# shreyaspadhy/CMCD

Hardware: AMD Instinct MI355X
Metric: bridge-steps*particles/sec (higher is better)
Workload: dtype f32; 1 GPU; many_gmm_n2000_k256_dds; model=many_gmm, boundmode=MCD_CAIS_sn, particles_per_gpu=2000, nbridges=256, nn_arch=dds, dim=2, global_particles=2000, parallelism=particles sharded x1, stats all-gather

## Files before the change

### cmcd_amd/csrc/cmcd_kernels.hip

```cpp
#include <hip/hip_runtime.h>
#include <math.h>
#include <stdint.h>
#include <stdio.h>
#include <stdlib.h>
#include <string.h>

#include "cmcd_common.h"
#include "cmcd_device.h"
#include "cmcd_hip.h"
#include "cmcd_host.h"

namespace cmcd {

struct SchedArgs {
  const float* params;
  float* ws;
  cmcd_layout lay;
  WsLayout w;
  int32_t K, ngrid, eps_schedule;
  int64_t gridref_x, target_x;
  uint32_t stamp = 0;
};

__device__ __forceinline__ void prep_sched_body(const SchedArgs& a) {
  __shared__ float gy[40], gx[40], gm[40];
  const int G = a.ngrid;
  if (threadIdx.x <= G) gm[threadIdx.x] = a.params[a.lay.mgridref_y + threadIdx.x];
  __syncthreads();
  if (threadIdx.x == 0) {
    float v[33];
#pragma unroll
    for (int i = 0; i < 33; ++i) v[i] = gm[i < G + 1 ? i : G];
    float run = 0.f;
#pragma unroll
    for (int i = 0; i < 33; ++i) {
      if (i <= G) {
        run += v[i];
        gy[i + 1] = run;
      }
    }
    gy[0] = 0.f;
    gm[39] = run;
  }
  __syncthreads();
  if (threadIdx.x < G + 2) {
    const float tot = gm[39];
    if (threadIdx.x >= 1) gy[threadIdx.x] = gy[threadIdx.x] / tot;
    gx[threadIdx.x] = (float)threadIdx.x / (float)(G + 1);
  }
  __syncthreads();
  const float eps0 = a.params[a.lay.eps];
  for (int i = threadIdx.x; i < a.K; i += blockDim.x) {
    const float x = (float)(i + 1) / (float)(a.K + 1);
    int j = (int)(x * (float)(G + 1)) + 1;
    j = j < 1 ? 1 : (j > G + 1 ? G + 1 : j);
    while (j > 1 && gx[j - 1] > x) --j;
    while (j < G + 1 && gx[j] <= x) ++j;
    const float dx = gx[j] - gx[j - 1], df = gy[j] - gy[j - 1];
    a.ws[a.w.beta + i] = gy[j - 1] + ((x - gx[j - 1]) / dx) * df;
    float e;
    if (a.eps_schedule == CMCD_EPS_COS_SQ) {
      const float phase = (float)i / (float)a.K;
      const float cs = cosf((phase + 0.008f) / 1.008f * 0.5f * 3.14159265358979323846f);
      e = eps0 * (cs * cs);
    } else if (a.eps_schedule == CMCD_EPS_LINEAR) {
      e = (0.0001f - eps0) / (float)(a.K - 1) * (float)i + eps0;
    } else {
      e = eps0;
    }
    const float s = sqrtf(2.0f * e);
    a.ws[a.w.eps + i] = e;
    a.ws[a.w.sig + i] = s;
    a.ws[a.w.logsig + i] = logf(s);
    float* sc = a.ws + a.w.sched + 8 * (int64_t)i;
    sc[0] = a.ws[a.w.beta + i];
    sc[1] = e;
    sc[2] = s;
    sc[3] = logf(s) + kHalfLog2Pi;
    sc[4] = 1.0f / (2.0f * s * s);
    sc[5] = e * sc[0];
    sc[6] = e * (1.0f - sc[0]);
    sc[7] = i == 0 ? __uint_as_float(a.stamp) : 0.f;
  }
}

__global__ void prep_sched_kernel(SchedArgs a) { prep_sched_body(a); }

struct DdsPrepArgs {
  const float* params;
  float* ws;
  cmcd_layout lay;
  WsLayout w;
  int32_t D;
};

__device__ __forceinline__ void prep_dds_body(const DdsPrepArgs& a, int t) {
  __shared__ float e[128], h[64], tau[64], red[4][64];
  const int j = threadIdx.x & 63, q = threadIdx.x >> 6;
  const float* P = a.params;
  float wa[32], wb[16], wc[16];
#pragma unroll
  for (int k = 0; k < 32; ++k) wa[k] = P[a.lay.d_tw1 + (32 * q + k) * 64 + j];
#pragma unroll
  for (int k = 0; k < 16; ++k) wb[k] = P[a.lay.d_tw2 + (16 * q + k) * 64 + j];
#pragma unroll
  for (int k = 0; k < 16; ++k) wc[k] = P[a.lay.d_sw1 + (a.D + 16 * q + k) * 64 + j];
  const float ba = P[a.lay.d_tb1 + j], bb = P[a.lay.d_tb2 + j], bc = P[a.lay.d_sb1 + j];
  if (q == 0) {
    float cj;
    {
#pragma clang fp contract(off)
      const float sj = (float)j / 63.0f;
      const float lo_part = 0.1f * (1.0f - sj), hi_part = 100.0f * sj;
      cj = (j == 63) ? 100.0f : lo_part + hi_part;
    }
    const float arg = cj * (float)t + P[a.lay.d_phase + j];
    e[j] = sinf(arg);
    e[64 + j] = cosf(arg);
  }
  __syncthreads();
  float acc = 0.f;
#pragma unroll
  for (int k = 0; k < 32; ++k) acc = fmaf(e[32 * q + k], wa[k], acc);
  red[q][j] = acc;
  __syncthreads();
  if (q == 0) h[j] = gelu_exact(ba + ((red[0][j] + red[1][j]) + (red[2][j] + red[3][j])));
  __syncthreads();
  acc = 0.f;
#pragma unroll
  for (int k = 0; k < 16; ++k) acc = fmaf(h[16 * q + k], wb[k], acc);
  __syncthreads();
  red[q][j] = acc;
  __syncthreads();
  if (q == 0) tau[j] = bb + ((red[0][j] + red[1][j]) + (red[2][j] + red[3][j]));
  __syncthreads();
  acc = 0.f;
#pragma unroll
  for (int k = 0; k < 16; ++k) acc = fmaf(tau[16 * q + k], wc[k], acc);
  __syncthreads();
  red[q][j] = acc;
  __syncthreads();
  if (q == 0) a.ws[a.w.bias1 + (int64_t)t * 64 + j] = bc + ((red[0][j] + red[1][j]) + (red[2][j] + red[3][j]));
}

struct GefPrepArgs {
  const float* params;
  float* ws;
  cmcd_layout lay;
  WsLayout w;
  int32_t D, E, K;
};

__device__ __forceinline__ void prep_geffner_body(const GefPrepArgs& a, int row) {
  const int ie = row < a.K ? row : a.K - 1;
  const int in = a.D + a.E;
  const float* P = a.params;
  const float* emb = P + a.lay.g_emb + (int64_t)ie * a.E;
  for (int n = threadIdx.x; n < a.w.HP; n += blockDim.x) {
    float b = 0.f, u = 0.f;
    if (n < in) {
      b = P[a.lay.g_b1 + n];
      const float* wcol = P + a.lay.g_w1 + (int64_t)a.D * in + n;
      int j = 0;
      for (; j + 8 <= a.E; j += 8) {
        float wv[8];
#pragma unroll
        for (int q = 0; q < 8; ++q) wv[q] = wcol[(int64_t)(j + q) * in];
#pragma unroll
        for (int q = 0; q < 8; ++q) b = fmaf(emb[j + q], wv[q], b);
      }
      for (; j < a.E; ++j) b = fmaf(emb[j], wcol[(int64_t)j * in], b);
      u = n >= a.D ? emb[n - a.D] : 0.f;
    }
    a.ws[a.w.bias1 + (int64_t)row * a.w.HP + n] = b;
    a.ws[a.w.utab + (int64_t)row * a.w.HP + n] = u;
  }
}

struct PackArgs {
  const float* params;
  const float* tgt;
  float* ws;
  WsLayout w;
  int64_t o_w1, o_w2, o_b2, o_w3, o_b3, o_factor;
  int32_t D, IN;
  int32_t DO;
  int32_t target, n_mix;
  uint32_t stamp;
};

__device__ __forceinline__ void pack_weights_body(const PackArgs& a, int vblock, int nblocks) {
  const int HP = a.w.HP, T = a.w.T;
  const float* P = a.params;
  const int64_t tid = (int64_t)vblock * blockDim.x + threadIdx.x;
  const int64_t stride = (int64_t)nblocks * blockDim.x;
  const bool has_net = a.o_w2 >= 0;
  for (int64_t idx = tid; has_net && idx < (int64_t)HP * HP; idx += stride) {
    const int r = idx & 3, lane = (idx >> 2) & 63;
    const int tt = int(idx >> 8), t_out = tt % T, t_in = tt / T;
    const int kin = 16 * t_in + 4 * (lane >> 4) + r, nout = 16 * t_out + (lane & 15);
    a.ws[a.w.w2 + idx] = (kin < a.IN && nout < a.IN) ? P[a.o_w2 + (int64_t)kin * a.IN + nout] : 0.f;
    const int krow = 16 * t_in + (lane & 15), ncon = 16 * t_out + 4 * (lane >> 4) + r;
    a.ws[a.w.w2t + idx] = (krow < a.IN && ncon < a.IN) ? P[a.o_w2 + (int64_t)krow * a.IN + ncon] : 0.f;
  }
  for (int64_t idx = tid; has_net && idx < 2 * (int64_t)HP * HP; idx += stride) {
    const int lane = idx & 63, rest = int(idx >> 6), sq = rest % (HP / 2), wvq = rest / (HP / 2);
    int kin = sq + (HP / 2) * ((lane >> 3) & 1), nout = 16 * wvq + 4 * (lane >> 4) + (lane & 3);
    if (wvq == 8 && coop_tail4(T, a.IN)) {
      const int sl = (lane >> 3) & 7;
      kin = sq < coop_tail_len(sl) ? coop_tail_start(sl) + sq : a.IN;
      nout = 128 + (lane & 3);
    }
    a.ws[a.w.w2q + idx] = (kin < a.IN && nout < a.IN) ? P[a.o_w2 + (int64_t)kin * a.IN + nout] : 0.f;
  }
  for (int64_t idx = tid; has_net && idx < (int64_t)a.D * HP; idx += stride) {
    const int j = int(idx / HP), n = int(idx % HP);
    a.ws[a.w.w1z + idx] = n < a.IN ? P[a.o_w1 + (int64_t)j * a.IN + n] : 0.f;
  }
  for (int64_t idx = tid; has_net && idx < (int64_t)a.DO * HP; idx += stride) {
    const int j = int(idx / HP), n = int(idx % HP);
    a.ws[a.w.w3t + idx] = n < a.IN ? P[a.o_w3 + (int64_t)n * a.DO + j] : 0.f;
  }
  for (int64_t idx = tid; has_net && idx < HP; idx += stride) a.ws[a.w.b2 + idx] = idx < a.IN ? P[a.o_b2 + idx] : 0.f;
  for (int64_t idx = tid; idx < 16; idx += stride) {
    float v = 0.f;
    if (has_net && idx < a.DO) v = P[a.o_b3 + idx];
    if (idx == 15) v = a.o_factor >= 0 ? P[a.o_factor] : 1.0f;
    if (idx == 13) v = __uint_as_float(a.stamp);
    a.ws[a.w.b3 + idx] = v;
  }
  if (a.target == CMCD_TARGET_MANY_GMM) {
    for (int64_t idx = tid; idx < a.w.tgt_floats; idx += stride) {
      float v = 0.f;
      const float s = a.tgt[0];
      if (idx == 0) v = 1.0f / s;
      else if (idx == 1) v = -0.5f * 1.44269504088896340736f / (s * s);
      else if (idx == 2) v = __int_as_float(a.n_mix);
      else if (idx == 3) v = 1.44269504088896340736f * (-2.0f * (logf(s) + kHalfLog2Pi) - logf((float)a.n_mix));
      else if (idx >= 4 && idx < 4 + 2 * a.n_mix) v = a.tgt[1 + (idx - 4)];
      a.ws[a.w.tgt + idx] = v;
    }
  }
}

struct PrepArgs {
  SchedArgs sched;
  DdsPrepArgs dds;
  GefPrepArgs gef;
  PackArgs pack;
  int32_t K, arch, npack;
};

__global__ __launch_bounds__(256) void prep_fused_kernel(PrepArgs a) {
  const int b = blockIdx.x;
  if (b <= a.K) {
    if (a.arch < 0) return;
    if (a.arch == CMCD_ARCH_DDS) prep_dds_body(a.dds, b);
    else prep_geffner_body(a.gef, b);
  } else if (b == a.K + 1) {
    prep_sched_body(a.sched);
  } else {
    pack_weights_body(a.pack, b - a.K - 2, a.npack);
  }
}


template <int ARCH>
__device__ __forceinline__ float act(float pre) {
  return ARCH == CMCD_ARCH_DDS ? gelu_exact(pre) : softplus(pre);
}

#ifndef CMCD_TRAJ_ABL
#define CMCD_TRAJ_ABL 0
#endif
#ifndef CMCD_TRAJ_PF
#define CMCD_TRAJ_PF 1
#endif
template <int ARCH, int D, int T, bool PF = (CMCD_TRAJ_PF != 0)>
__device__ __forceinline__ void eval_net(const float (&z)[D], const float* __restrict__ brow,
                                         const float* __restrict__ urow, const float* lds_w2,
                                         const float* lds_w1z, const float* lds_b2, const float* lds_w3t,
                                         const float* lds_b3, int lane, float (&s)[D]) {
  constexpr int HP = 16 * T;
  const int g = lane >> 4;
  asm volatile("" ::: "memory");
  f32x4 h[T];
#pragma unroll
  for (int t = 0; t < T; ++t) {
    f32x4 pre = *reinterpret_cast<const f32x4*>(brow + 16 * t + 4 * g);
#pragma unroll
    for (int j = 0; j < D; ++j) {
      const f32x4 wv = *reinterpret_cast<const f32x4*>(lds_w1z + j * HP + 16 * t + 4 * g);
      pre += z[j] * wv;
    }
    if (ARCH == CMCD_ARCH_DDS) {
#pragma unroll
      for (int r = 0; r < 4; ++r) h[t][r] = (CMCD_TRAJ_ABL & 2) ? pre[r] : gelu_fast(pre[r]);
    } else {
      f32x4 u = *reinterpret_cast<const f32x4*>(urow + 16 * t + 4 * g);
      if (16 * t < D) {
#pragma unroll
        for (int r = 0; r < 4; ++r) {
          const int nidx = 16 * t + 4 * g + r;
#pragma unroll
          for (int j = 0; j < D; ++j)
            if (j >= 16 * t && j < 16 * t + 16) u[r] = (nidx == j) ? z[j] : u[r];
        }
      }
#pragma unroll
      for (int r = 0; r < 4; ++r) h[t][r] = u[r] + softplus(pre[r]);
    }
  }
  float dummy = z[0];
  f32x4 acc[T];
#pragma unroll
  for (int t = 0; t < T; ++t) acc[t] = *reinterpret_cast<const f32x4*>(lds_b2 + 16 * t + 4 * g);
  if (PF) {
    f32x4 a[2][T];
    asm volatile("" ::: "memory");
#pragma unroll
    for (int to = 0; to < T; ++to) a[0][to] = *reinterpret_cast<const f32x4*>(lds_w2 + (to * 64 + lane) * 4);
#pragma unroll
    for (int ti = 0; ti < T; ++ti) {
      asm volatile("" ::: "memory");
      if (ti + 1 < T) {
#pragma unroll
        for (int to = 0; to < T; ++to)
          a[(ti + 1) & 1][to] = *reinterpret_cast<const f32x4*>(lds_w2 + (((ti + 1) * T + to) * 64 + lane) * 4);
      }
      __builtin_amdgcn_sched_barrier(0);
#pragma unroll
      for (int r = 0; r < 4; ++r) {
#pragma unroll
        for (int to = 0; to < T; ++to)
          acc[to] = __builtin_amdgcn_mfma_f32_16x16x4f32(a[ti & 1][to][r], h[ti][r], acc[to], 0, 0, 0);
      }
      __builtin_amdgcn_sched_barrier(0);
    }
  } else {
#pragma unroll
  for (int ti = 0; ti < T; ++ti) {
    asm volatile("" ::: "memory");
    f32x4 a[T];
#pragma unroll
    for (int to = 0; to < T; ++to)
      a[to] = *reinterpret_cast<const f32x4*>(lds_w2 + ((ti * T + to) * 64 + lane) * 4);
#pragma unroll
    for (int r = 0; r < 4; ++r) {
#pragma unroll
      for (int to = 0; to < T; ++to) {
        if (CMCD_TRAJ_ABL & 1) acc[to][r] += a[to][r] * h[ti][r];
        else acc[to] = __builtin_amdgcn_mfma_f32_16x16x4f32(a[to][r], h[ti][r], acc[to], 0, 0, 0);
      }
      if (CMCD_TRAJ_ABL & 16) {
#pragma unroll
        for (int q = 0; q < 24; ++q) asm volatile("v_fma_f32 %0, %0, %1, %1" : "+v"(dummy) : "v"(z[0]));
      }
    }
  }
  }
  if (CMCD_TRAJ_ABL & 32) {
#pragma unroll
    for (int q = 0; q < 24 * 4 * T; ++q) asm volatile("v_fma_f32 %0, %0, %1, %1" : "+v"(dummy) : "v"(z[0]));
  }
  float part[D];
#pragma unroll
  for (int j = 0; j < D; ++j) part[j] = 0.f;
#pragma unroll
  for (int t = 0; t < T; ++t) {
    f32x4 h2;
#pragma unroll
    for (int r = 0; r < 4; ++r)
      h2[r] = (ARCH == CMCD_ARCH_DDS) ? ((CMCD_TRAJ_ABL & 2) ? acc[t][r] : gelu_fast(acc[t][r])) : h[t][r] + softplus(acc[t][r]);
#pragma unroll
    for (int j = 0; j < D; ++j) {
      const f32x4 wv = *reinterpret_cast<const f32x4*>(lds_w3t + j * HP + 16 * t + 4 * g);
      part[j] += h2[0] * wv[0] + h2[1] * wv[1] + h2[2] * wv[2] + h2[3] * wv[3];
    }
  }
  const float factor = lds_b3[15];
#pragma unroll
  for (int j = 0; j < D; ++j) {
    const float o = group_sum(part[j]) + lds_b3[j];
    s[j] = (ARCH == CMCD_ARCH_DDS) ? fminf(fmaxf(o, -1e4f), 1e4f) : o * factor;
  }
  if (CMCD_TRAJ_ABL & 48) s[0] += dummy * 1e-30f;
}

__device__ __forceinline__ float traj_rs32(float x, float y) {
  uint32_t r0, r1;
  swap32(__float_as_uint(x), __float_as_uint(y), r0, r1);
  return __uint_as_float(r0) + __uint_as_float(r1);
}
__device__ __forceinline__ float traj_rs16(float x, float y) {
  uint32_t r0, r1;
  swap16(__float_as_uint(x), __float_as_uint(y), r0, r1);
  return __uint_as_float(r0) + __uint_as_float(r1);
}
template <int ARCH, int D, int T>
__device__ __forceinline__ void eval_net_tail4(const float (&z)[D], const float* __restrict__ brow,
                                               const float* __restrict__ urow, const float* lds_w2,
                                               const float* lds_w1z, const float* lds_b2, const float* lds_w3t,
                                               const float* lds_b3, int lane, float (&s)[D]) {
  static_assert(ARCH == CMCD_ARCH_GEFFNER && T >= 2 && D <= 16, "the tail form is the geffner net's");
  constexpr int HP = 16 * T, TF = T - 1, NX = 16 * TF;
  const int g = lane >> 4, c = lane & 15;
  asm volatile("" ::: "memory");
  f32x4 h[TF];
#pragma unroll
  for (int t = 0; t < TF; ++t) {
    f32x4 pre = *reinterpret_cast<const f32x4*>(brow + 16 * t + 4 * g);
#pragma unroll
    for (int j = 0; j < D; ++j) {
      const f32x4 wv = *reinterpret_cast<const f32x4*>(lds_w1z + j * HP + 16 * t + 4 * g);
      pre += z[j] * wv;
    }
    f32x4 u = *reinterpret_cast<const f32x4*>(urow + 16 * t + 4 * g);
    if (16 * t < D) {
#pragma unroll
      for (int r = 0; r < 4; ++r) {
        const int nidx = 16 * t + 4 * g + r;
#pragma unroll
        for (int j = 0; j < D; ++j)
          if (j >= 16 * t && j < 16 * t + 16) u[r] = (nidx == j) ? z[j] : u[r];
      }
    }
#pragma unroll
    for (int r = 0; r < 4; ++r) h[t][r] = u[r] + softplus(pre[r]);
  }
  float hx;
  {
    float px = brow[NX + g];
#pragma unroll
    for (int j = 0; j < D; ++j) px = fmaf(z[j], lds_w1z[j * HP + NX + g], px);
    hx = urow[NX + g] + softplus(px);
  }
  f32x4 acc[TF], accx = {0.f, 0.f, 0.f, 0.f};
#pragma unroll
  for (int t = 0; t < TF; ++t) acc[t] = *reinterpret_cast<const f32x4*>(lds_b2 + 16 * t + 4 * g);
  const float* const w2x = lds_w2 + (TF * 64 + 16 * g + (c & 3)) * 4;
  {
    f32x4 a[2][TF], ax[2];
    asm volatile("" ::: "memory");
#pragma unroll
    for (int to = 0; to < TF; ++to) a[0][to] = *reinterpret_cast<const f32x4*>(lds_w2 + (to * 64 + lane) * 4);
    ax[0] = *reinterpret_cast<const f32x4*>(w2x);
#pragma unroll
    for (int ti = 0; ti < TF; ++ti) {
      asm volatile("" ::: "memory");
      if (ti + 1 < TF) {
#pragma unroll
        for (int to = 0; to < TF; ++to)
          a[(ti + 1) & 1][to] = *reinterpret_cast<const f32x4*>(lds_w2 + (((ti + 1) * T + to) * 64 + lane) * 4);
        ax[(ti + 1) & 1] = *reinterpret_cast<const f32x4*>(w2x + (ti + 1) * T * 256);
      }
      __builtin_amdgcn_sched_barrier(0);
#pragma unroll
      for (int r = 0; r < 4; ++r) {
#pragma unroll
        for (int to = 0; to < TF; ++to)
          acc[to] = __builtin_amdgcn_mfma_f32_16x16x4f32(a[ti & 1][to][r], h[ti][r], acc[to], 0, 0, 0);
        accx = __builtin_amdgcn_mfma_f32_4x4x1f32(ax[ti & 1][r], h[ti][r], accx, 0, 0, 0);
      }
      __builtin_amdgcn_sched_barrier(0);
    }
  }
  {
    float a8[TF];
#pragma unroll
    for (int to = 0; to < TF; ++to) a8[to] = lds_w2[((TF * T + to) * 64 + c) * 4 + g];
    const float axx = lds_w2[((TF * T + TF) * 64 + (c & 3)) * 4 + g];
#pragma unroll
    for (int to = 0; to < TF; ++to) acc[to] = __builtin_amdgcn_mfma_f32_16x16x4f32(a8[to], hx, acc[to], 0, 0, 0);
    accx = __builtin_amdgcn_mfma_f32_4x4x1f32(axx, hx, accx, 0, 0, 0);
  }
  float h2x;
  {
    const float u01 = traj_rs16(accx[0], accx[1]), u23 = traj_rs16(accx[2], accx[3]);
    const float avx = traj_rs32(u01, u23) + lds_b2[NX + g];
    h2x = hx + softplus(avx);
  }
  float part[D];
#pragma unroll
  for (int j = 0; j < D; ++j) part[j] = h2x * lds_w3t[j * HP + NX + g];
#pragma unroll
  for (int t = 0; t < TF; ++t) {
    f32x4 h2;
#pragma unroll
    for (int r = 0; r < 4; ++r) h2[r] = h[t][r] + softplus(acc[t][r]);
#pragma unroll
    for (int j = 0; j < D; ++j) {
      const f32x4 wv = *reinterpret_cast<const f32x4*>(lds_w3t + j * HP + 16 * t + 4 * g);
      part[j] += h2[0] * wv[0] + h2[1] * wv[1] + h2[2] * wv[2] + h2[3] * wv[3];
    }
  }
  const float factor = lds_b3[15];
#pragma unroll
  for (int j = 0; j < D; ++j) s[j] = (group_sum(part[j]) + lds_b3[j]) * factor;
}

constexpr bool traj_pf(int ARCH, int D, int T) {
  return CMCD_TRAJ_PF != 0 && (T == 9 || (D == 2 && (T == 2 || ARCH == CMCD_ARCH_DDS)));
}
#ifndef CMCD_TRAJ_TAIL4
#define CMCD_TRAJ_TAIL4 1
#endif
template <int TARGET, int ARCH, int D, int T, bool PF = traj_pf(ARCH, D, T), bool TAIL4 = false>
__global__ __launch_bounds__(512, (T > 4 || D > 4) ? 2 : 4) void traj_kernel(TrajArgs a) {
  constexpr int HP = 16 * T;
  extern __shared__ __attribute__((aligned(16))) float lds[];
  float* lds_w2 = lds;
  float* lds_w1z = lds_w2 + HP * HP;
  float* lds_w3t = lds_w1z + D * HP;
  float* lds_b2 = lds_w3t + D * HP;
  float* lds_b3 = lds_b2 + HP;
  float* lds_tgt = lds_b3 + 16;
  {
    const f32x4* src = reinterpret_cast<const f32x4*>(a.ws + a.w.w1z);
    f32x4* dst = reinterpret_cast<f32x4*>(lds_w1z);
    for (int i = threadIdx.x; i < D * HP / 4; i += blockDim.x) dst[i] = src[i];
    src = reinterpret_cast<const f32x4*>(a.ws + a.w.w2);
    dst = reinterpret_cast<f32x4*>(lds_w2);
    for (int i = threadIdx.x; i < HP * HP / 4; i += blockDim.x) dst[i] = src[i];
    src = reinterpret_cast<const f32x4*>(a.ws + a.w.w3t);
    dst = reinterpret_cast<f32x4*>(lds_w3t);
    for (int i = threadIdx.x; i < D * HP / 4; i += blockDim.x) dst[i] = src[i];
    for (int i = threadIdx.x; i < HP; i += blockDim.x) lds_b2[i] = a.ws[a.w.b2 + i];
    for (int i = threadIdx.x; i < 16; i += blockDim.x) lds_b3[i] = a.ws[a.w.b3 + i];
    for (int i = threadIdx.x; i < a.w.tgt_floats; i += blockDim.x) lds_tgt[i] = a.ws[a.w.tgt + i];
    float warm = 0.f;
    const int64_t t0 = a.w.sched;
    const int64_t t1 = (ARCH == CMCD_ARCH_GEFFNER ? a.w.utab : a.w.bias1) + (int64_t)(a.K + 1) * HP;
    const int64_t per_xcd = (gridDim.x + 7) >> 3, rank = blockIdx.x >> 3;
    for (int64_t i = t0 + 32 * (rank * blockDim.x + threadIdx.x); i < t1; i += 32 * per_xcd * blockDim.x) warm += a.ws[i];
    asm volatile("" ::"v"(warm));
  }
  __syncthreads();

  const int lane = threadIdx.x & 63, g = lane >> 4, c = lane & 15;
  const int64_t wave = (int64_t)blockIdx.x * (blockDim.x >> 6) + (threadIdx.x >> 6);
  if (wave * 16 >= a.n) return;
  const int64_t p = wave * 16 + c;
  const bool valid = p < a.n;
  const int32_t seed = a.seeds[valid ? p : a.n - 1];
  const int K = a.K;

  float qmean[D], qstd[D], qiv[D];
#pragma unroll
  for (int j = 0; j < D; ++j) {
    qmean[j] = a.params[a.lay.vd_mean + j];
    qstd[j] = expf(a.params[a.lay.vd_logdiag + j]);
    qiv[j] = 1.0f / (qstd[j] * qstd[j]);
  }

  const int gb = g & 1;
  uint32_t x0, x1, k0 = 0u, k1 = (uint32_t)seed;
  float z[D];
  {
    x0 = gb; x1 = 2 + gb;
    threefry2x32(k0, k1, x0, x1);
    uint32_t a0, a1, b0, b1;
    rows01(x0, a0, a1);
    rows01(x1, b0, b1);
    constexpr int Hh = (D + 1) / 2;
    float nz[2 * Hh];
#pragma unroll
    for (int j0 = 0; j0 < Hh; j0 += 4) {
      const int j = j0 + g;
      uint32_t y0 = j, y1 = (Hh + j < D) ? Hh + j : 0;
      threefry2x32(a0, a1, y0, y1);
      if (a.dbg_bits && valid && j < Hh) {
        a.dbg_bits[p * D + j] = y0;
        a.dbg_noise[p * D + j] = bits_to_normal(y0);
        if (Hh + j < D) {
          a.dbg_bits[p * D + Hh + j] = y1;
          a.dbg_noise[p * D + Hh + j] = bits_to_normal(y1);
        }
      }
      uint32_t r0[4], r1[4];
      rows0123(__float_as_uint(bits_to_normal(y0)), r0);
      rows0123(__float_as_uint(bits_to_normal(y1)), r1);
#pragma unroll
      for (int q = 0; q < 4; ++q)
        if (j0 + q < Hh) {
          nz[j0 + q] = __uint_as_float(r0[q]);
          nz[Hh + j0 + q] = __uint_as_float(r1[q]);
        }
    }
#pragma unroll
    for (int j = 0; j < D; ++j) z[j] = qstd[j] * nz[j] + qmean[j];
    if (a.traj && valid && g == 0) {
#pragma unroll
      for (int j = 0; j < D; ++j) a.traj[p * D + j] = z[j];
    }
    x0 = gb; x1 = 2 + gb;
    threefry2x32(b0, b1, x0, x1);
    uint32_t c0, c1;
    rows01(x0, c0, c1);
    x0 = gb; x1 = 2 + gb;
    threefry2x32(c0, c1, x0, x1);
    rows01(x1, k0, k1);
    if (a.dbg_keys && valid && g == 0) {
      a.dbg_keys[p * 2] = k0;
      a.dbg_keys[p * 2 + 1] = k1;
    }
  }

  float w = 0.f;
#pragma unroll
  for (int j = 0; j < D; ++j) {
    const float dz = z[j] - qmean[j];
    w -= -(dz * dz) / (2.0f * qstd[j] * qstd[j]) - logf(qstd[j]) - kHalfLog2Pi;
  }

  const float clipv = a.var_mode ? 1e2f : 1e3f;
  const bool clip_p = a.grad_clipping != 0;
  const bool clip_q = clip_p && a.var_mode;

  const float* bias1 = a.ws + a.w.bias1;
  const float* utab = a.ws + a.w.utab;

  float zp[D];
  float fk_lp = 0.f;
  float pbeta = 0.f, peps = 0.f, pinv2s2 = 0.f, pcst = 0.f;
  float logp = 0.f;
#pragma unroll
  for (int j = 0; j < D; ++j) zp[j] = 0.f;

  for (int i = 0; i <= K; ++i) {
    float gp[D], sn[D];
    if (CMCD_TRAJ_ABL & 4) {
#pragma unroll
      for (int j = 0; j < D; ++j) gp[j] = -z[j];
      logp = z[0];
    } else {
      Target<TARGET, D>::eval(z, g, lds_tgt, logp, gp);
    }
    if (a.ula == 1) {
#pragma unroll
      for (int j = 0; j < D; ++j) sn[j] = 0.f;
    } else {
      const int64_t row = (a.ula == 2) ? (i > 0 ? i - 1 : 0) : i;
      if constexpr (TAIL4) eval_net_tail4<ARCH, D, T>(z, bias1 + row * HP, utab + row * HP, lds_w2, lds_w1z, lds_b2, lds_w3t, lds_b3, lane, sn);
      else eval_net<ARCH, D, T, PF>(z, bias1 + row * HP, utab + row * HP, lds_w2, lds_w1z, lds_b2, lds_w3t, lds_b3, lane, sn);
    }
    const float fsn = a.ula ? 0.f : 1.f;
    float gq[D];
#pragma unroll
    for (int j = 0; j < D; ++j) {
      gq[j] = -(z[j] - qmean[j]) * qiv[j];
      if (clip_p) gp[j] = fminf(fmaxf(gp[j], -clipv), clipv);
      if (clip_q) gq[j] = fminf(fmaxf(gq[j], -clipv), clipv);
    }

    if (i > 0) {
      float bk_lp = 0.f;
#pragma unroll
      for (int j = 0; j < D; ++j) {
        const float ub = -1.0f * (pbeta * gp[j] + (1.0f - pbeta) * gq[j]);
        const float bk = z[j] - peps * ub + peps * sn[j];
        const float db = zp[j] - bk;
        bk_lp += -(db * db) * pinv2s2 - pcst;
      }
      w += bk_lp - fk_lp;
    }
    if (i == K) break;

    const float* scr = a.ws + a.w.sched + 8 * (int64_t)i;
    const float beta = scr[0], eps = scr[1], sig = scr[2], cst = scr[3], inv2s2 = scr[4];

    x0 = gb; x1 = 2 + gb;
    threefry2x32(k0, k1, x0, x1);
    uint32_t g0, g1, h0, h1;
    rows01(x0, g0, g1);
    rows01(x1, h0, h1);
    constexpr int Hh = (D + 1) / 2;
    constexpr int NB = 2 + Hh;
    float nz[2 * Hh];
#pragma unroll
    for (int b0 = 0; b0 < NB; b0 += 4) {
      const int b = b0 + g;
      const bool is_split = b < 2;
      const int jn = b - 2;
      uint32_t y0 = is_split ? b : jn;
      uint32_t y1 = is_split ? 2 + b : ((Hh + jn < D) ? Hh + jn : 0);
      if (!(CMCD_TRAJ_ABL & 8)) threefry2x32(is_split ? h0 : g0, is_split ? h1 : g1, y0, y1);
      if (b0 == 0) {
        rows01(y1, k0, k1);
        if (a.dbg_keys && valid && g == 0) {
          a.dbg_keys[((int64_t)(i + 1) * a.n + p) * 2] = k0;
          a.dbg_keys[((int64_t)(i + 1) * a.n + p) * 2 + 1] = k1;
        }
      }
      if (a.dbg_bits && valid && jn >= 0 && jn < Hh) {
        const int64_t o = ((int64_t)(i + 1) * a.n + p) * D;
        a.dbg_bits[o + jn] = y0;
        a.dbg_noise[o + jn] = bits_to_normal(y0);
        if (Hh + jn < D) {
          a.dbg_bits[o + Hh + jn] = y1;
          a.dbg_noise[o + Hh + jn] = bits_to_normal(y1);
        }
      }
      if (D == 2 && !(CMCD_TRAJ_ABL & 8)) {
        uint32_t t0, t1;
        swap16(y1, y1, t0, t1);
        const float dev = bits_to_normal(g == 3 ? t0 : y0);
        uint32_t rr[4];
        rows0123(__float_as_uint(dev), rr);
        nz[0] = __uint_as_float(rr[2]);
        nz[1] = __uint_as_float(rr[3]);
      } else {
        uint32_t r0[4], r1[4];
        rows0123(__float_as_uint((CMCD_TRAJ_ABL & 8) ? __uint_as_float(y0) * 1e-9f : bits_to_normal(y0)), r0);
        rows0123(__float_as_uint((CMCD_TRAJ_ABL & 8) ? __uint_as_float(y1) * 1e-9f : bits_to_normal(y1)), r1);
#pragma unroll
        for (int q = 0; q < 4; ++q) {
          const int jj = b0 + q - 2;
          if (jj >= 0 && jj < Hh) {
            nz[jj] = __uint_as_float(r0[q]);
            nz[Hh + jj] = __uint_as_float(r1[q]);
          }
        }
      }
    }

    fk_lp = 0.f;
#pragma unroll
    for (int j = 0; j < D; ++j) {
      const float uf = -1.0f * (beta * gp[j] + (1.0f - beta) * gq[j]);
      const float fk = z[j] - eps * uf - eps * (fsn * sn[j]);
      const float zn = fk + sig * nz[j];
      const float df = zn - fk;
      fk_lp += -(df * df) * inv2s2 - cst;
      zp[j] = z[j];
      z[j] = zn;
    }
    if (a.traj && valid && g == 0) {
#pragma unroll
      for (int j = 0; j < D; ++j) a.traj[((int64_t)(i + 1) * a.n + p) * D + j] = z[j];
    }
    pbeta = beta; peps = eps; pinv2s2 = inv2s2; pcst = cst;
  }
  w += logp;
  const float loss = -w;

  if (valid && g == 0) {
    a.out_loss[p] = loss;
#pragma unroll
    for (int j = 0; j < D; ++j) a.out_z[p * D + j] = z[j];
  }

  const bool use = valid && g == 0;
  double cnt = (use && isfinite(loss)) ? 1.0 : 0.0;
  double sm = use ? (double)loss : 0.0;
  double sq = use ? (double)loss * (double)loss : 0.0;
  double mx = use ? -(double)loss : -INFINITY;
#pragma unroll
  for (int o = 1; o < 16; o <<= 1) {
    cnt += __shfl_xor(cnt, o);
    sm += __shfl_xor(sm, o);
    sq += __shfl_xor(sq, o);
    mx = fmax(mx, __shfl_xor(mx, o));
  }
  double ex = (use && mx > -INFINITY && mx < INFINITY) ? exp(-(double)loss - mx) : 0.0;
#pragma unroll
  for (int o = 1; o < 16; o <<= 1) ex += __shfl_xor(ex, o);
  if (lane == 0) {
    double* o = a.partials + wave * CMCD_NSTATS;
    o[0] = cnt; o[1] = sm; o[2] = sq; o[3] = mx; o[4] = ex;
  }
}

__device__ __forceinline__ void stats_merge(double* a, const double* b) {
  a[0] += b[0];
  a[1] += b[1];
  a[2] += b[2];
  const double m = fmax(a[3], b[3]);
  const double sa = (a[3] > -INFINITY && m < INFINITY) ? a[4] * exp(a[3] - m) : (a[3] == m ? a[4] : 0.0);
  const double sb = (b[3] > -INFINITY && m < INFINITY) ? b[4] * exp(b[3] - m) : (b[3] == m ? b[4] : 0.0);
  a[3] = m;
  a[4] = sa + sb;
}

__global__ __launch_bounds__(256) void finalize_kernel(const double* partials, int32_t n_waves, double* out,
                                                       const uint32_t* stamp_slot = nullptr, uint32_t stamp_expect = 0) {
  __shared__ double shm[256];
  __shared__ double sh[256][4];
  const int per = (n_waves + 255) / 256;
  const int lo = threadIdx.x * per, hi = min(n_waves, lo + per);
  double m = -INFINITY;
  for (int i = lo; i < hi; ++i) m = fmax(m, partials[(int64_t)i * CMCD_NSTATS + 3]);
  shm[threadIdx.x] = m;
  __syncthreads();
  for (int s = 128; s > 0; s >>= 1) {
    if (threadIdx.x < s) shm[threadIdx.x] = fmax(shm[threadIdx.x], shm[threadIdx.x + s]);
    __syncthreads();
  }
  const double M = shm[0];
  double acc[4] = {0, 0, 0, 0};
  for (int i = lo; i < hi; ++i) {
    const double* p = partials + (int64_t)i * CMCD_NSTATS;
    acc[0] += p[0];
    acc[1] += p[1];
    acc[2] += p[2];
    acc[3] += (p[3] > -INFINITY && M < INFINITY) ? p[4] * exp(p[3] - M) : (p[3] == M ? p[4] : 0.0);
  }
  for (int k = 0; k < 4; ++k) sh[threadIdx.x][k] = acc[k];
  __syncthreads();
  for (int s = 128; s > 0; s >>= 1) {
    if (threadIdx.x < s)
      for (int k = 0; k < 4; ++k) sh[threadIdx.x][k] += sh[threadIdx.x + s][k];
    __syncthreads();
  }
  if (threadIdx.x == 0) {
    out[0] = sh[0][0];
    out[1] = sh[0][1];
    out[2] = sh[0][2];
    out[3] = M;
    out[4] = sh[0][3];
    if (stamp_slot && *stamp_slot != stamp_expect)
      for (int k = 0; k < CMCD_NSTATS; ++k) out[k] = __builtin_nan("");
  }
}

__global__ void vargrad_weights_kernel(const float* loss, const double* stats, int64_t n, int64_t n_total,
                                       float* omega) {
  const int64_t i = (int64_t)blockIdx.x * blockDim.x + threadIdx.x;
  if (i >= n) return;
  const double mean = stats[1] / (double)n_total;
  const double var = stats[2] / (double)n_total - mean * mean;
  const bool clipped = var > 1e7 || var < -1e7;
  omega[i] = (var != var) ? __builtin_nanf("") : (clipped ? 0.0f : (float)(-2.0 / (double)n_total * ((double)loss[i] - mean)));
}

typedef void (*traj_fn)(TrajArgs);

template <int TARGET, int ARCH, int D>
static traj_fn pick_T(int T) {
  switch (T) {
    case 2: return traj_kernel<TARGET, ARCH, D, 2>;
    case 4: return traj_kernel<TARGET, ARCH, D, 4>;
    case 9: return traj_kernel<TARGET, ARCH, D, 9>;
    default: return nullptr;
  }
}

static bool traj_tail4(const cmcd_desc& d, int T) {
  const int in = net_in_dim(d) + d.emb_dim;
  return CMCD_TRAJ_TAIL4 != 0 && d.arch == CMCD_ARCH_GEFFNER && d.dim == 2 && T == 9 && in > 128 && in <= 132 &&
         (d.target == CMCD_TARGET_MANY_GMM || d.target == CMCD_TARGET_GMM);
}

static traj_fn pick_kernel(const cmcd_desc& d, int T) {
  if (traj_tail4(d, T)) {
    constexpr bool pf = traj_pf(CMCD_ARCH_GEFFNER, 2, 9);
    return d.target == CMCD_TARGET_MANY_GMM ? traj_kernel<CMCD_TARGET_MANY_GMM, CMCD_ARCH_GEFFNER, 2, 9, pf, true>
                                            : traj_kernel<CMCD_TARGET_GMM, CMCD_ARCH_GEFFNER, 2, 9, pf, true>;
  }
  if (d.arch == CMCD_ARCH_DDS) {
    if (T != 4) return nullptr;
    if (d.target == CMCD_TARGET_MANY_GMM && d.dim == 2) return traj_kernel<CMCD_TARGET_MANY_GMM, CMCD_ARCH_DDS, 2, 4>;
    if (d.target == CMCD_TARGET_GMM && d.dim == 2) return traj_kernel<CMCD_TARGET_GMM, CMCD_ARCH_DDS, 2, 4>;
    if (d.target == CMCD_TARGET_FUNNEL && d.dim == 10) return traj_kernel<CMCD_TARGET_FUNNEL, CMCD_ARCH_DDS, 10, 4>;
    return nullptr;
  }
  if (d.target == CMCD_TARGET_MANY_GMM && d.dim == 2) return pick_T<CMCD_TARGET_MANY_GMM, CMCD_ARCH_GEFFNER, 2>(T);
  if (d.target == CMCD_TARGET_GMM && d.dim == 2) return pick_T<CMCD_TARGET_GMM, CMCD_ARCH_GEFFNER, 2>(T);
  if (d.target == CMCD_TARGET_FUNNEL && d.dim == 10) return pick_T<CMCD_TARGET_FUNNEL, CMCD_ARCH_GEFFNER, 10>(T);
  return nullptr;
}

bool traj_available(const cmcd_desc& d, int T) { return pick_kernel(d, T) != nullptr; }

int traj_launch(const cmcd_desc& d, const WsLayout& w, const TrajArgs& ta, hipStream_t stream,
                int (*before_launch)(hipStream_t)) {
  traj_fn fn = pick_kernel(d, w.T);
  const int64_t tiles = w.n_waves, D = d.dim;
  const size_t lds_bytes = size_t(w.HP * w.HP + 2 * D * w.HP + w.HP + 16 + w.tgt_floats) * 4;
  if (lds_bytes > 160 * 1024) return fail(CMCD_ERR_UNSUPPORTED, "network too wide for LDS%s");
  int64_t per_cu = (160 * 1024) / (int64_t)lds_bytes;
  int nw = tiles <= 1024 ? 1 : (tiles <= 8192 ? 4 : 8);
  if (per_cu < 2 && tiles > 256) nw = tiles <= 1024 ? 4 : 8;
  CMCD_HIP_CHECK(hipFuncSetAttribute(reinterpret_cast<const void*>(fn),
                                     hipFuncAttributeMaxDynamicSharedMemorySize, (int)lds_bytes));
  const unsigned blocks = unsigned((tiles + nw - 1) / nw);
  const int rc = before_launch ? before_launch(stream) : CMCD_OK;
  if (rc != CMCD_OK) return rc;
  hipLaunchKernelGGL(fn, dim3(blocks), dim3(64 * nw), lds_bytes, stream, ta);
  return CMCD_OK;
}

void launch_prep_sched(const cmcd_desc& d, const cmcd_layout& lay, const WsLayout& w, const float* params, float* ws,
                       hipStream_t stream, uint32_t stamp) {
  SchedArgs sa{params, ws, lay, w, d.nbridges, d.ngrid, d.eps_schedule, -1, -1};
  sa.stamp = stamp;
  hipLaunchKernelGGL(prep_sched_kernel, dim3(1), dim3(256), 0, stream, sa);
}

void launch_prep(const cmcd_desc& d, const cmcd_layout& layr, const WsLayout& w, const float* params,
                 const float* target_consts, int n_mix, float* ws, hipStream_t stream, uint32_t stamp) {
  const cmcd_layout* lay = &layr;
  const int64_t K = d.nbridges, D = net_in_dim(d), E = d.emb_dim, IN = D + E;
  PrepArgs pa{};
  pa.sched = SchedArgs{params, ws, *lay, w, (int32_t)K, d.ngrid, d.eps_schedule, -1, -1};
  PackArgs& pk = pa.pack;
  pk.stamp = stamp;
  pa.sched.stamp = stamp;
  pk.params = params; pk.tgt = target_consts; pk.ws = ws; pk.w = w;
  pk.D = (int32_t)D; pk.DO = d.dim; pk.target = d.target; pk.n_mix = n_mix;
  if (d.mode == CMCD_MODE_ULA) {
    pk.o_w1 = pk.o_w2 = pk.o_b2 = pk.o_w3 = pk.o_b3 = pk.o_factor = -1; pk.IN = 0;
  } else if (d.arch == CMCD_ARCH_DDS) {
    pa.dds = DdsPrepArgs{params, ws, *lay, w, (int32_t)D};
    pk.o_w1 = lay->d_sw1; pk.o_w2 = lay->d_sw2; pk.o_b2 = lay->d_sb2; pk.o_w3 = lay->d_sw3;
    pk.o_b3 = lay->d_sb3; pk.o_factor = -1; pk.IN = 64;
  } else {
    pa.gef = GefPrepArgs{params, ws, *lay, w, (int32_t)D, (int32_t)E, (int32_t)K};
    pk.o_w1 = lay->g_w1; pk.o_w2 = lay->g_w2; pk.o_b2 = lay->g_b2; pk.o_w3 = lay->g_w3;
    pk.o_b3 = lay->g_b3; pk.o_factor = lay->g_factor; pk.IN = (int32_t)IN;
  }
  pa.K = (int32_t)K; pa.arch = d.mode == CMCD_MODE_ULA ? -1 : d.arch;
  pa.npack = (w.HP * w.HP + 255) / 256;
  if (pa.npack > 64) pa.npack = 64;
  hipLaunchKernelGGL(prep_fused_kernel, dim3((unsigned)(K + 2 + pa.npack)), dim3(256), 0, stream, pa);
}

void launch_finalize(const double* partials, int32_t count, double* out5, hipStream_t stream, const uint32_t* stamp_slot,
                     uint32_t stamp) {
  hipLaunchKernelGGL(finalize_kernel, dim3(1), dim3(256), 0, stream, partials, count, out5, stamp_slot, stamp);
}

int launch_finalize(const double* partials, int32_t count, double* out5, void* stream) {
  launch_finalize(partials, count, out5, static_cast<hipStream_t>(stream), nullptr, 0u);
  return hipGetLastError() == hipSuccess ? CMCD_OK : fail(CMCD_ERR_HIP, "finalize launch failed%s");
}

void launch_vargrad_weights(const float* loss, const double* stats, int64_t n, int64_t n_total, float* omega,
                            hipStream_t stream) {
  hipLaunchKernelGGL(vargrad_weights_kernel, dim3((unsigned)((n + 255) / 256)), dim3(256), 0, stream, loss, stats, n, n_total,
                     omega);
}

}
```

Measured before the change: 2.761 billion bridge-steps*particles/s.

## Streamline prep and finalize kernels with lane broadcasts and wave reductions

The DDS time-embedding prep now has every wave compute sin/cos itself and broadcasts values with readlane instead of staging them in shared memory, which cuts the number of block barriers. The pack-weights loops rotate their starting thread so small tail loops spread across threads, and the pack block count is sized from the total packed work. The finalize kernel swaps its shared-memory tree reductions for wave shuffles and can keep up to four partial records in registers. A compile-time ablation macro is added to skip prep sections. These are small launch-overhead kernels, so the effect on end-to-end throughput is likely small, and the float summation order in finalize changes.

```diff
diff --git a/cmcd_amd/csrc/cmcd_kernels.hip b/cmcd_amd/csrc/cmcd_kernels.hip
--- a/cmcd_amd/csrc/cmcd_kernels.hip
+++ b/cmcd_amd/csrc/cmcd_kernels.hip
@@ -94,9 +94,13 @@
   int32_t D;
 };
 
+__device__ __forceinline__ float lane_value(float v, int l) {
+  return __int_as_float(__builtin_amdgcn_readlane(__float_as_int(v), l));
+}
+
 __device__ __forceinline__ void prep_dds_body(const DdsPrepArgs& a, int t) {
-  __shared__ float e[128], h[64], tau[64], red[4][64];
-  const int j = threadIdx.x & 63, q = threadIdx.x >> 6;
+  __shared__ float red[3][4][64];
+  const int j = threadIdx.x & 63, q = __builtin_amdgcn_readfirstlane(threadIdx.x >> 6);
   const float* P = a.params;
   float wa[32], wb[16], wc[16];
 #pragma unroll
@@ -106,41 +110,37 @@
 #pragma unroll
   for (int k = 0; k < 16; ++k) wc[k] = P[a.lay.d_sw1 + (a.D + 16 * q + k) * 64 + j];
   const float ba = P[a.lay.d_tb1 + j], bb = P[a.lay.d_tb2 + j], bc = P[a.lay.d_sb1 + j];
-  if (q == 0) {
-    float cj;
-    {
+  const float phase = P[a.lay.d_phase + j];
+  float cj;
+  {
 #pragma clang fp contract(off)
-      const float sj = (float)j / 63.0f;
-      const float lo_part = 0.1f * (1.0f - sj), hi_part = 100.0f * sj;
-      cj = (j == 63) ? 100.0f : lo_part + hi_part;
-    }
-    const float arg = cj * (float)t + P[a.lay.d_phase + j];
-    e[j] = sinf(arg);
-    e[64 + j] = cosf(arg);
-  }
+    const float sj = (float)j / 63.0f;
+    const float lo_part = 0.1f * (1.0f - sj), hi_part = 100.0f * sj;
+    cj = (j == 63) ? 100.0f : lo_part + hi_part;
+  }
+  const float arg = cj * (float)t + phase;
+  const float sn = sinf(arg), cs = cosf(arg);
+  const float ev = q < 2 ? sn : cs;
+  const int e0 = 32 * (q & 1), h0 = 16 * q;
+  auto quarters = [&](int c) { return (red[c][0][j] + red[c][1][j]) + (red[c][2][j] + red[c][3][j]); };
+  float acc = 0.f;
+#pragma unroll
+  for (int k = 0; k < 32; ++k) acc = fmaf(lane_value(ev, e0 + k), wa[k], acc);
+  red[0][q][j] = acc;
   __syncthreads();
-  float acc = 0.f;
-#pragma unroll
-  for (int k = 0; k < 32; ++k) acc = fmaf(e[32 * q + k], wa[k], acc);
-  red[q][j] = acc;
+  const float hv = gelu_exact(ba + quarters(0));
+  acc = 0.f;
+#pragma unroll
+  for (int k = 0; k < 16; ++k) acc = fmaf(lane_value(hv, h0 + k), wb[k], acc);
+  red[1][q][j] = acc;
   __syncthreads();
-  if (q == 0) h[j] = gelu_exact(ba + ((red[0][j] + red[1][j]) + (red[2][j] + red[3][j])));
+  const float tv = bb + quarters(1);
+  acc = 0.f;
+#pragma unroll
+  for (int k = 0; k < 16; ++k) acc = fmaf(lane_value(tv, h0 + k), wc[k], acc);
+  red[2][q][j] = acc;
   __syncthreads();
-  acc = 0.f;
-#pragma unroll
-  for (int k = 0; k < 16; ++k) acc = fmaf(h[16 * q + k], wb[k], acc);
-  __syncthreads();
-  red[q][j] = acc;
-  __syncthreads();
-  if (q == 0) tau[j] = bb + ((red[0][j] + red[1][j]) + (red[2][j] + red[3][j]));
-  __syncthreads();
-  acc = 0.f;
-#pragma unroll
-  for (int k = 0; k < 16; ++k) acc = fmaf(tau[16 * q + k], wc[k], acc);
-  __syncthreads();
-  red[q][j] = acc;
-  __syncthreads();
-  if (q == 0) a.ws[a.w.bias1 + (int64_t)t * 64 + j] = bc + ((red[0][j] + red[1][j]) + (red[2][j] + red[3][j]));
+  if (q == 0) a.ws[a.w.bias1 + (int64_t)t * 64 + j] = bc + quarters(2);
 }
 
 struct GefPrepArgs {
@@ -195,15 +195,24 @@
   const int64_t tid = (int64_t)vblock * blockDim.x + threadIdx.x;
   const int64_t stride = (int64_t)nblocks * blockDim.x;
   const bool has_net = a.o_w2 >= 0;
-  for (int64_t idx = tid; has_net && idx < (int64_t)HP * HP; idx += stride) {
+  const uint32_t nthr = (uint32_t)stride;
+  uint32_t base = 0;
+  auto first = [&](int64_t n) {
+    const int64_t f = tid - (int64_t)base;
+    base = (base + (uint32_t)(n % nthr)) % nthr;
+    return f < 0 ? f + stride : f;
+  };
+  for (int64_t idx = first(has_net ? (int64_t)HP * HP : 0); has_net && idx < (int64_t)HP * HP; idx += stride) {
     const int r = idx & 3, lane = (idx >> 2) & 63;
     const int tt = int(idx >> 8), t_out = tt % T, t_in = tt / T;
     const int kin = 16 * t_in + 4 * (lane >> 4) + r, nout = 16 * t_out + (lane & 15);
-    a.ws[a.w.w2 + idx] = (kin < a.IN && nout < a.IN) ? P[a.o_w2 + (int64_t)kin * a.IN + nout] : 0.f;
     const int krow = 16 * t_in + (lane & 15), ncon = 16 * t_out + 4 * (lane >> 4) + r;
-    a.ws[a.w.w2t + idx] = (krow < a.IN && ncon < a.IN) ? P[a.o_w2 + (int64_t)krow * a.IN + ncon] : 0.f;
-  }
-  for (int64_t idx = tid; has_net && idx < 2 * (int64_t)HP * HP; idx += stride) {
+    const float v = (kin < a.IN && nout < a.IN) ? P[a.o_w2 + (int64_t)kin * a.IN + nout] : 0.f;
+    const float vt = (krow < a.IN && ncon < a.IN) ? P[a.o_w2 + (int64_t)krow * a.IN + ncon] : 0.f;
+    a.ws[a.w.w2 + idx] = v;
+    a.ws[a.w.w2t + idx] = vt;
+  }
+  for (int64_t idx = first(has_net ? 2 * (int64_t)HP * HP : 0); has_net && idx < 2 * (int64_t)HP * HP; idx += stride) {
     const int lane = idx & 63, rest = int(idx >> 6), sq = rest % (HP / 2), wvq = rest / (HP / 2);
     int kin = sq + (HP / 2) * ((lane >> 3) & 1), nout = 16 * wvq + 4 * (lane >> 4) + (lane & 3);
     if (wvq == 8 && coop_tail4(T, a.IN)) {
@@ -213,16 +222,16 @@
     }
     a.ws[a.w.w2q + idx] = (kin < a.IN && nout < a.IN) ? P[a.o_w2 + (int64_t)kin * a.IN + nout] : 0.f;
   }
-  for (int64_t idx = tid; has_net && idx < (int64_t)a.D * HP; idx += stride) {
+  for (int64_t idx = first(has_net ? (int64_t)a.D * HP : 0); has_net && idx < (int64_t)a.D * HP; idx += stride) {
     const int j = int(idx / HP), n = int(idx % HP);
     a.ws[a.w.w1z + idx] = n < a.IN ? P[a.o_w1 + (int64_t)j * a.IN + n] : 0.f;
   }
-  for (int64_t idx = tid; has_net && idx < (int64_t)a.DO * HP; idx += stride) {
+  for (int64_t idx = first(has_net ? (int64_t)a.DO * HP : 0); has_net && idx < (int64_t)a.DO * HP; idx += stride) {
     const int j = int(idx / HP), n = int(idx % HP);
     a.ws[a.w.w3t + idx] = n < a.IN ? P[a.o_w3 + (int64_t)n * a.DO + j] : 0.f;
   }
-  for (int64_t idx = tid; has_net && idx < HP; idx += stride) a.ws[a.w.b2 + idx] = idx < a.IN ? P[a.o_b2 + idx] : 0.f;
-  for (int64_t idx = tid; idx < 16; idx += stride) {
+  for (int64_t idx = first(has_net ? HP : 0); has_net && idx < HP; idx += stride) a.ws[a.w.b2 + idx] = idx < a.IN ? P[a.o_b2 + idx] : 0.f;
+  for (int64_t idx = first(16); idx < 16; idx += stride) {
     float v = 0.f;
     if (has_net && idx < a.DO) v = P[a.o_b3 + idx];
     if (idx == 15) v = a.o_factor >= 0 ? P[a.o_factor] : 1.0f;
@@ -230,7 +239,7 @@
     a.ws[a.w.b3 + idx] = v;
   }
   if (a.target == CMCD_TARGET_MANY_GMM) {
-    for (int64_t idx = tid; idx < a.w.tgt_floats; idx += stride) {
+    for (int64_t idx = first(a.w.tgt_floats); idx < a.w.tgt_floats; idx += stride) {
       float v = 0.f;
       const float s = a.tgt[0];
       if (idx == 0) v = 1.0f / s;
@@ -251,8 +260,12 @@
   int32_t K, arch, npack;
 };
 
+#ifndef CMCD_PREP_ABL
+#define CMCD_PREP_ABL 0
+#endif
 __global__ __launch_bounds__(256) void prep_fused_kernel(PrepArgs a) {
   const int b = blockIdx.x;
+  if (CMCD_PREP_ABL & (b <= a.K ? 1 : (b == a.K + 1 ? 2 : 4))) return;
   if (b <= a.K) {
     if (a.arch < 0) return;
     if (a.arch == CMCD_ARCH_DDS) prep_dds_body(a.dds, b);
@@ -782,44 +795,83 @@
   a[4] = sa + sb;
 }
 
+constexpr int kFinHold = 4;
+
+__device__ __forceinline__ double fin_tree_sum(double x) {
+#pragma unroll
+  for (int o = 32; o > 0; o >>= 1) x += __shfl_down(x, o);
+  return x;
+}
+__device__ __forceinline__ double fin_wave_max(double x) {
+#pragma unroll
+  for (int o = 32; o > 0; o >>= 1) x = fmax(x, __shfl_xor(x, o));
+  return x;
+}
+
 __global__ __launch_bounds__(256) void finalize_kernel(const double* partials, int32_t n_waves, double* out,
                                                        const uint32_t* stamp_slot = nullptr, uint32_t stamp_expect = 0) {
-  __shared__ double shm[256];
-  __shared__ double sh[256][4];
+  __shared__ double shm[4];
+  __shared__ double sh[3][4][64];
+  const int lane = threadIdx.x & 63, wv = threadIdx.x >> 6;
+  const uint32_t stamp_seen = stamp_slot ? *stamp_slot : stamp_expect;
   const int per = (n_waves + 255) / 256;
   const int lo = threadIdx.x * per, hi = min(n_waves, lo + per);
+  const bool held = per <= kFinHold;
+  double rec[kFinHold][CMCD_NSTATS];
   double m = -INFINITY;
-  for (int i = lo; i < hi; ++i) m = fmax(m, partials[(int64_t)i * CMCD_NSTATS + 3]);
-  shm[threadIdx.x] = m;
+  if (held) {
+#pragma unroll
+    for (int q = 0; q < kFinHold; ++q) {
+      const bool use = lo + q < hi;
+      const double* p = partials + (int64_t)(lo + q) * CMCD_NSTATS;
+#pragma unroll
+      for (int k = 0; k < CMCD_NSTATS; ++k) rec[q][k] = use ? p[k] : (k == 3 ? -INFINITY : 0.0);
+    }
+#pragma unroll
+    for (int q = 0; q < kFinHold; ++q) m = fmax(m, rec[q][3]);
+  } else {
+    for (int i = lo; i < hi; ++i) m = fmax(m, partials[(int64_t)i * CMCD_NSTATS + 3]);
+  }
+  m = fin_wave_max(m);
+  if (lane == 0) shm[wv] = m;
   __syncthreads();
-  for (int s = 128; s > 0; s >>= 1) {
-    if (threadIdx.x < s) shm[threadIdx.x] = fmax(shm[threadIdx.x], shm[threadIdx.x + s]);
-    __syncthreads();
-  }
-  const double M = shm[0];
+  const double M = fmax(fmax(shm[0], shm[1]), fmax(shm[2], shm[3]));
   double acc[4] = {0, 0, 0, 0};
-  for (int i = lo; i < hi; ++i) {
-    const double* p = partials + (int64_t)i * CMCD_NSTATS;
-    acc[0] += p[0];
-    acc[1] += p[1];
-    acc[2] += p[2];
-    acc[3] += (p[3] > -INFINITY && M < INFINITY) ? p[4] * exp(p[3] - M) : (p[3] == M ? p[4] : 0.0);
-  }
-  for (int k = 0; k < 4; ++k) sh[threadIdx.x][k] = acc[k];
+  auto add = [&](double p0, double p1, double p2, double p3, double p4) {
+    acc[0] += p0;
+    acc[1] += p1;
+    acc[2] += p2;
+    acc[3] += (p3 > -INFINITY && M < INFINITY) ? p4 * exp(p3 - M) : (p3 == M ? p4 : 0.0);
+  };
+  if (held) {
+#pragma unroll
+    for (int q = 0; q < kFinHold; ++q)
+      if (lo + q < hi) add(rec[q][0], rec[q][1], rec[q][2], rec[q][3], rec[q][4]);
+  } else {
+    for (int i = lo; i < hi; ++i) {
+      const double* p = partials + (int64_t)i * CMCD_NSTATS;
+      add(p[0], p[1], p[2], p[3], p[4]);
+    }
+  }
+  if (wv > 0) {
+#pragma unroll
+    for (int k = 0; k < 4; ++k) sh[wv - 1][k][lane] = acc[k];
+  }
   __syncthreads();
-  for (int s = 128; s > 0; s >>= 1) {
-    if (threadIdx.x < s)
-      for (int k = 0; k < 4; ++k) sh[threadIdx.x][k] += sh[threadIdx.x + s][k];
-    __syncthreads();
-  }
-  if (threadIdx.x == 0) {
-    out[0] = sh[0][0];
-    out[1] = sh[0][1];
-    out[2] = sh[0][2];
-    out[3] = M;
-    out[4] = sh[0][3];
-    if (stamp_slot && *stamp_slot != stamp_expect)
-      for (int k = 0; k < CMCD_NSTATS; ++k) out[k] = __builtin_nan("");
+  if (wv > 0) return;
+  double v[4];
+#pragma unroll
+  for (int k = 0; k < 4; ++k) {
+    const double a0 = acc[k] + sh[1][k][lane], a1 = sh[0][k][lane] + sh[2][k][lane];
+    v[k] = fin_tree_sum(a0 + a1);
+  }
+  if (lane == 0) {
+    const bool refused = stamp_seen != stamp_expect;
+    out[0] = refused ? __builtin_nan("") : v[0];
+    out[1] = refused ? __builtin_nan("") : v[1];
+    out[2] = refused ? __builtin_nan("") : v[2];
+    out[3] = refused ? __builtin_nan("") : M;
+    out[4] = refused ? __builtin_nan("") : v[3];
   }
 }
 
@@ -920,7 +972,8 @@
     pk.o_b3 = lay->g_b3; pk.o_factor = lay->g_factor; pk.IN = (int32_t)IN;
   }
   pa.K = (int32_t)K; pa.arch = d.mode == CMCD_MODE_ULA ? -1 : d.arch;
-  pa.npack = (w.HP * w.HP + 255) / 256;
+  const int64_t packed = (d.mode != CMCD_MODE_ULA ? 3 * (int64_t)w.HP * w.HP + (D + d.dim + 1) * (int64_t)w.HP : 0) + 16 + w.tgt_floats;
+  pa.npack = (int32_t)((packed + 255) / 256);
   if (pa.npack > 64) pa.npack = 64;
   hipLaunchKernelGGL(prep_fused_kernel, dim3((unsigned)(K + 2 + pa.npack)), dim3(256), 0, stream, pa);
 }
```

New measurement: 2.762 billion bridge-steps*particles/s (median of 2 runs). Within noise of the previous version (+0.1%).
